# facebookresearch/lightplane

Measured on AMD Instinct MI355X. Metric: Mrays/sec fwd+bwd, 64^3x16ch triplane @128 samples; peak bwd mem (MB), higher is better.
Workload: dtype f32

## Files before the change

lightplane_amd/csrc/lp_bf3.h:

```cpp
#pragma once
#include "lp_mfma_common.h"

namespace lp {

typedef __bf16 bf16x2_t __attribute__((ext_vector_type(2)));
typedef __bf16 bf16x8_t __attribute__((ext_vector_type(8)));
typedef float f32x2_t __attribute__((ext_vector_type(2)));
typedef unsigned u32x4_t __attribute__((ext_vector_type(4)));

#define LP_MFMA_BF16(a, b, c) \
  __builtin_amdgcn_mfma_f32_32x32x16_bf16(__builtin_bit_cast(bf16x8_t, (a)), __builtin_bit_cast(bf16x8_t, (b)), (c), 0, 0, 0)

LP_DEV unsigned pk_bf16(float a, float b) {
  const f32x2_t v = {a, b};
  return __builtin_bit_cast(unsigned, __builtin_convertvector(v, bf16x2_t));
}
LP_DEV float bf16_lo(unsigned p) { return __builtin_bit_cast(float, p << 16); }
LP_DEV float bf16_hi(unsigned p) { return __builtin_bit_cast(float, p & 0xffff0000u); }

LP_DEV void split3_scalar(float x, unsigned short& l1, unsigned short& l2, unsigned short& l3) {
  const unsigned p1 = pk_bf16(x, 0.0f);
  const float r1 = x - bf16_lo(p1);
  const unsigned p2 = pk_bf16(r1, 0.0f);
  const float r2 = r1 - bf16_lo(p2);
// ... 110 lines not shown
  return acc;
}
LP_DEV void split2_chunk(const float* v, u32x4_t& l1, u32x4_t& l2) {
#pragma unroll
  for (int i = 0; i < 4; ++i) {
    const float a = v[2 * i], b = v[2 * i + 1];
    const unsigned p1 = pk_bf16(a, b);
    l1[i] = p1;
    l2[i] = pk_bf16(a - bf16_lo(p1), b - bf16_hi(p1));
  }
}
template <class A>
LP_DEV f32x16 chunk_bf2(const A& a, int c, int lane, const u32x4_t& l1, const u32x4_t& l2, f32x16 acc) {
  {
    const u32x4_t w2 = a(c, 1, lane);
    acc = LP_MFMA_BF16(w2, l1, acc);
  }
  {
    const u32x4_t w1 = a(c, 0, lane);
    acc = LP_MFMA_BF16(w1, l2, acc);
    acc = LP_MFMA_BF16(w1, l1, acc);
  }
  return acc;
}
template <int NCH, class A>
LP_DEV f32x16 layer_bf2v(const A& a, int lane, const float (&v)[8 * NCH], f32x16 acc, char* trow = nullptr) {
  u32x4_t l1, l2;
  split2_chunk(v, l1, l2);
#pragma unroll
  for (int c = 0; c < NCH; ++c) {
    u32x4_t n1 = l1, n2 = l2;
    if (trow) {
      *reinterpret_cast<u32x4_t*>(trow + 32 * c) = l1;
      *reinterpret_cast<u32x4_t*>(trow + 32 * c + rm_bytes(32)) = l2;
    }
    acc = chunk_bf2(a, c, lane, l1, l2, acc);
    if (c + 1 < NCH) split2_chunk(v + 8 * (c + 1), n1, n2);
    l1 = n1; l2 = n2;
  }
  return acc;
}
template <int NCH>
LP_DEV void limb_tile_store(char* trow, const float (&v)[8 * NCH]) {
#pragma unroll
  for (int c = 0; c < NCH; ++c) {
    u32x4_t l1, l2;
    float w[8];
#pragma unroll
    for (int i = 0; i < 8; ++i) {
      w[i] = v[8 * c + i];
      asm volatile("" : "+v"(w[i]));
    }
    split2_chunk(w, l1, l2);
    *reinterpret_cast<u32x4_t*>(trow + 32 * c) = l1;
    *reinterpret_cast<u32x4_t*>(trow + 32 * c + rm_bytes(32)) = l2;
  }
}

template <int DXL>
LP_DEV void dx_split_chunk(const float* v, u32x4_t& l1, u32x4_t& l2, u32x4_t& l3) {
  if constexpr (DXL == 2) {
    split2_chunk(v, l1, l2);
    l3 = l2;
  } else {
    split3_chunk(v, l1, l2, l3);
  }
}
template <int DXL, class A>
LP_DEV f32x16 dx_chunk(const A& a, int c, int lane, const u32x4_t& l1, const u32x4_t& l2, const u32x4_t& l3, f32x16 acc) {
  if constexpr (DXL == 2) return chunk_bf2(a, c, lane, l1, l2, acc);
  else return chunk_bf3(a, c, lane, l1, l2, l3, acc);
}
template <int NCH, int DXL = 2, class A>
LP_DEV f32x16 layer_dxv(const A& a, int lane, const float (&v)[8 * NCH], f32x16 acc, char* trow = nullptr) {
  if constexpr (DXL == 2) return layer_bf2v<NCH>(a, lane, v, acc, trow);
  else return layer_bf3v<NCH>(a, lane, v, acc);
}

template <int NCH>
LP_DEV f32x16 layer_bf3v(const char* img, int chunk0, int lane, const float (&v)[8 * NCH], f32x16 acc) {
  return layer_bf3v<NCH>(ASlots{img, chunk0}, lane, v, acc);
}

template <int NCH, class A1, class A2>
LP_DEV void layer2_bf3v(const A1& a1, const A2& a2, int lane, const float (&v)[8 * NCH], f32x16& acc_a, f32x16& acc_b) {
  u32x4_t l1, l2, l3;
  split3_chunk(v, l1, l2, l3);
#pragma unroll
  for (int c = 0; c < NCH; ++c) {
    u32x4_t n1 = l1, n2 = l2, n3 = l3;
    acc_a = chunk_bf3(a1, c, lane, l1, l2, l3, acc_a);
    acc_b = chunk_bf3(a2, c, lane, l1, l2, l3, acc_b);
    if (c + 1 < NCH) {
      split3_chunk(v + 8 * (c + 1), n1, n2, n3);
      bf3_interleave_hint();
    }
    l1 = n1; l2 = n2; l3 = n3;
  }
}
template <int NCH>
LP_DEV void layer2_bf3v(const char* img, int chunk_a, int chunk_b, int lane, const float (&v)[8 * NCH], f32x16& acc_a,
                        f32x16& acc_b) {
  layer2_bf3v<NCH>(ASlots{img, chunk_a}, ASlots{img, chunk_b}, lane, v, acc_a, acc_b);
}

template <bool FWD>
// ... 131 lines not shown
```

lightplane_amd/csrc/lp_device.h:

```cpp
#pragma once

#include <hip/hip_runtime.h>
#include <stdint.h>

#include "../../include/lightplane_hip.h"

#define LP_DEV __device__ __forceinline__

namespace lp {


struct Ray {
  float ox, oy, oz, dx, dy, dz, near_t, far_t;
  int b;
};

LP_DEV Ray load_ray(const LpRays& r, int64_t i) {
  Ray q;
  q.ox = r.origins[3 * i + 0];
  q.oy = r.origins[3 * i + 1];
  q.oz = r.origins[3 * i + 2];
  q.dx = r.directions[3 * i + 0];
  q.dy = r.directions[3 * i + 1];
  q.dz = r.directions[3 * i + 2];
// ... 308 lines not shown
    const int U = (xy || xz) ? g.W : g.H;
    const int V = xy ? g.H : g.D;
    int iu, iv;
    float wu[2], wv[2];
    bool oku[2], okv[2];
    axis_taps<SPLAT>(cu, U, iu, wu, oku);
    axis_taps<SPLAT>(cv, V, iv, wv, okv);
    t.n = 4;
    t.su = 1; t.sv = U; t.st = 0;
    t.row0 = base + iv * U + iu;
    t.iu = iu;
    t.cell = 0;
    t.ok = 0;
#pragma unroll
    for (int k = 0; k < 4; ++k) {
      const int uu = k & 1, uv = (k >> 1) & 1;
      const bool ok = oku[uu] && okv[uv];
      t.ok |= ok ? (1u << k) : 0u;
      t.w[k] = ok ? wu[uu] * wv[uv] : 0.0f;
    }
#pragma unroll
    for (int k = 4; k < 8; ++k) t.w[k] = 0.0f;
  }
}

LP_DEV float scaffold_lookup(const float* scaffold, const LpGrid& s, int b, float x, float y, float z) {
  if (!point_in_bounds(x, y, z)) return 0.0f;
  const float fx = rintf(unnormalize<false>(x, s.W));
  const float fy = rintf(unnormalize<false>(y, s.H));
  const float fz = rintf(unnormalize<false>(z, s.D));
  if (!(fx >= 0.0f && fx <= (float)(s.W - 1) && fy >= 0.0f && fy <= (float)(s.H - 1) && fz >= 0.0f &&
        fz <= (float)(s.D - 1)))
    return 0.0f;
  const int64_t row = (((int64_t)b * s.D + (int)fz) * s.H + (int)fy) * s.W + (int)fx;
  return scaffold[row];
}


LP_DEV float softplus_f(float x) {
  const float e = __expf(x);
  const float series = e * fmaf(e, fmaf(e, 0.333333343f, -0.5f), 1.0f);
  const float lg = __logf(1.0f + e);
  const float sp = (e < 0.015625f) ? series : lg;
  return (x > 20.0f) ? x : sp;
}
LP_DEV float relu_f(float x) {
  const int i = __builtin_bit_cast(int, x);
  return __builtin_bit_cast(float, i > 0 ? i : 0);
}

LP_DEV unsigned mask_bit(unsigned m, float relu_value, int q) {
  return m | ((relu_value > 0.0f) ? (1u << q) : 0u);
}
LP_DEV float mask_apply(unsigned m, int q, float v) {
  const int all = ((int)(m << (31 - q))) >> 31;
  return __builtin_bit_cast(float, __builtin_bit_cast(int, v) & all);
}

LP_DEV float sigmoid_f(float x) { return __builtin_amdgcn_rcpf(1.0f + __expf(-x)); }
LP_DEV float d_softplus_f(float x) { return (x > 20.0f) ? 1.0f : sigmoid_f(x); }


LP_DEV int32_t hash32(int32_t x) {
  x = (int32_t)((uint32_t)((x >> 16) ^ x) * 0x45D9F3Bu);
  x = (int32_t)((uint32_t)((x >> 16) ^ x) * 0x45D9F3Bu);
  return (x >> 16) ^ x;
}
LP_DEV int32_t pair_hash(int32_t x, int32_t h) {
  const uint32_t u = (uint32_t)(h ^ x);
  return (int32_t)((u << 24) + u * 0x193u);
}
LP_DEV float int32_to_u01(int32_t h) {
  return (((float)h + 2147483648.0f) + 3.0f) / 4294967296.0f;
}
LP_DEV float hash_randn(int32_t x1, int32_t x2, int32_t seed) {
  const int32_t prime = 105097564;
  const int32_t h1 = pair_hash(pair_hash(prime, seed), hash32(x1));
  const int32_t h2 = pair_hash(pair_hash(prime, seed + 1), hash32(x2));
  const float u1 = int32_to_u01(h1), u2 = int32_to_u01(h2);
  return sqrtf(-2.0f * logf(u1)) * cosf(6.28318530718f * u2);
}
LP_DEV float sample_noise(int64_t ray, int step, int64_t n_rays, int s_tot, int32_t seed) {
  const int64_t i1 = ray * s_tot + step + 1;
  const int64_t pad = n_rays > 16 ? n_rays : 16;
  const int64_t i2 = i1 + pad * s_tot;
  return hash_randn((int32_t)(uint32_t)(uint64_t)i1, (int32_t)(uint32_t)(uint64_t)i2, seed);
}

LP_DEV void write_ray_outputs(const LpRendererArgs& a, int64_t ray_id, float len, float nlt, const float* facc) {
  a.ray_length[ray_id] = len;
  a.neg_log_t[ray_id] = nlt;
  const bool epi = a.bg_color != nullptr || a.alpha != nullptr;
  const float T = epi ? expf(-nlt) : 0.0f;
  for (int c = 0; c < a.color_chn; ++c) {
    float f = facc[c];
    if (a.bg_color) f = f + T * a.bg_color[c];
    a.feature[ray_id * a.color_chn + c] = f;
  }
  if (a.alpha) a.alpha[ray_id] = (a.alpha_mode == 2) ? -nlt : 1.0f - T;
}
LP_DEV float epilogue_grad_nlt(const LpRendererArgs& a, int64_t rid, bool valid, float nlt_final, float g_nlt,
                               const float* gfeat, int n_chn) {
  if (a.bg_color == nullptr && a.grad_alpha == nullptr) return g_nlt;
  const float T = expf(-nlt_final);
  if (a.grad_alpha && valid) {
    const float ga = a.grad_alpha[rid];
// ... 20 lines not shown
```

lightplane_amd/csrc/lp_mfma_common.h:

```cpp
#pragma once
#include <stdlib.h>

#include "lp_device.h"
#include "lp_splat_walk.h"
#include "lp_host.h"
#include "lp_plane_range.h"

namespace lp {

typedef float f32x16 __attribute__((ext_vector_type(16)));

LP_DEV constexpr int featq(int q, int h) { return (q & 3) + 8 * (q >> 2) + 4 * h; }

#define LP_MFMA(a, b, c) __builtin_amdgcn_mfma_f32_32x32x2f32((a), (b), (c), 0, 0, 0)

LP_DEV int opaque_zero() {
  int z = 0;
  asm volatile("" : "+s"(z));
  return z;
}

constexpr int HID = 32;
constexpr int W_LD = 33;
constexpr int WAVES = 4;
// ... 66 lines not shown
  if (!plain || S > RANGE_MAX_S || __ballot(!valid) != 0) return w;
  const LpGrid* g = a.grid.grids;
  const int W = g[0].W, H = g[0].H, D = (GM == GM_TRIPLANE) ? g[1].D : g[0].D;
  const AxisSpans ax = ray_axis_spans(ray.ox, ray.oy, ray.oz, ray.dx, ray.dy, ray.dz, ray.near_t, ray.far_t, S, W, H, D);
#pragma unroll
  for (int p = 0; p < (GM == GM_TRIPLANE ? 3 : 1); ++p) {
    const SampleSpan sp = (GM == GM_TRIPLANE) ? plane_span(ax, p, S) : voxel_span(ax, S);
    const int lo = wave_min_i(sp.lo), hi = -wave_min_i(-sp.hi);
    if (p == 0) w.lo3 = w.hi3 = 0u;
    w.lo3 |= (unsigned)(hi < lo ? 511 : lo) << (10 * p);
    w.hi3 |= (unsigned)(hi < lo ? 0 : hi) << (10 * p);
  }
  if (GM == GM_VOXEL) {
    w.lo3 *= 0x00100401u;
    w.hi3 *= 0x00100401u;
  }
  w.lo3 = (unsigned)__builtin_amdgcn_readfirstlane((int)w.lo3);
  w.hi3 = (unsigned)__builtin_amdgcn_readfirstlane((int)w.hi3);
  return w;
}

template <int C>
LP_DEV void gather_tap(const float* data, int row, float w, int h, float (&x0)[C / 2]) {
  const float4* src = reinterpret_cast<const float4*>(data + (int64_t)(row < 0 ? 0 : row) * C + 4 * h);
#pragma unroll
  for (int j = 0; j < C / 8; ++j) {
    const float4 v = src[2 * j];
    x0[4 * j + 0] = fmaf(w, v.x, x0[4 * j + 0]);
    x0[4 * j + 1] = fmaf(w, v.y, x0[4 * j + 1]);
    x0[4 * j + 2] = fmaf(w, v.z, x0[4 * j + 2]);
    x0[4 * j + 3] = fmaf(w, v.w, x0[4 * j + 3]);
  }
}

template <int C>
LP_DEV void gather_taps4(const float* data, const int* row, const float* w, float keep, int h, float (&x0)[C / 2]) {
  float4 v[4][C / 8];
#pragma unroll
  for (int k = 0; k < 4; ++k) {
    const float4* src = reinterpret_cast<const float4*>(data + (int64_t)(row[k] < 0 ? 0 : row[k]) * C + 4 * h);
#pragma unroll
    for (int j = 0; j < C / 8; ++j) v[k][j] = src[2 * j];
  }
  __builtin_amdgcn_sched_barrier(0);
#pragma unroll
  for (int k = 0; k < 4; ++k) {
    const float wk = w[k] * keep;
#pragma unroll
    for (int j = 0; j < C / 8; ++j) {
      x0[4 * j + 0] = fmaf(wk, v[k][j].x, x0[4 * j + 0]);
      x0[4 * j + 1] = fmaf(wk, v[k][j].y, x0[4 * j + 1]);
      x0[4 * j + 2] = fmaf(wk, v[k][j].z, x0[4 * j + 2]);
      x0[4 * j + 3] = fmaf(wk, v[k][j].w, x0[4 * j + 3]);
    }
  }
}

template <int C, bool FENCED>
LP_DEV void gather_list(const LpGridList& gl, bool mask_oob, const Ray& ray, float x, float y, float z, int h,
                        float (&x0)[C / 2]) {
#pragma unroll
  for (int q = 0; q < C / 2; ++q) x0[q] = 0.0f;
  const float keep = (mask_oob && !point_in_bounds(x, y, z)) ? 0.0f : 1.0f;
  for (int g = 0; g < gl.n_grids; ++g) {
    Taps t;
    const float* data = gl.grids[g].data;
    grid_taps<false>(gl.grids[g], ray.b, x, y, z, t);
    if (FENCED) __builtin_amdgcn_sched_barrier(0);
    gather_taps4<C>(data, t.row, t.w, keep, h, x0);
    if (FENCED) __builtin_amdgcn_sched_barrier(0);
    if (t.n == 8) {
      gather_taps4<C>(data, t.row + 4, t.w + 4, keep, h, x0);
      if (FENCED) __builtin_amdgcn_sched_barrier(0);
    }
  }
}

template <int C, int GM, bool FENCED = false>
LP_DEV void gather_features(const LpRendererArgs& a, const Ray& ray, float x, float y, float z, int h,
                            float (&x0)[C / 2], unsigned pm = WaveRanges::G) {
#pragma unroll
  for (int q = 0; q < C / 2; ++q) x0[q] = 0.0f;
  const float keep = (a.march.mask_out_of_bounds && !point_in_bounds(x, y, z)) ? 0.0f : 1.0f;
  if (GM == GM_TRIPLANE) {
    if (FENCED) {
      AxisTap ax, ay, az;
      triplane_axes<false>(a.grid.grids, x, y, z, ax, ay, az);
      const int W = a.grid.grids[0].W, H = a.grid.grids[0].H, D = a.grid.grids[1].D;
#pragma unroll
      for (int g = 0; g < 3; ++g) {
        __builtin_amdgcn_sched_barrier(0);
        if (pm & WaveRanges::bit(g)) {
          Taps t;
          plane_taps_from_axes((int)a.grid.grids[g].row_offset + ray.b * ((g == 0 ? H : D) * (g == 2 ? H : W)), g == 2 ? H : W,
                               g == 2 ? ay : ax, g == 0 ? ay : az, t);
          gather_taps4<C>(a.grid.grids[g].data, t.row, t.w, keep, h, x0);
        }
      }
      __builtin_amdgcn_sched_barrier(0);
    } else {
      Taps t[3];
      triplane_taps<false>(a.grid.grids, ray.b, x, y, z, t);
#pragma unroll
      for (int g = 0; g < 3; ++g) {
        if (!(pm & WaveRanges::bit(g))) continue;
#pragma unroll
        for (int k = 0; k < 4; ++k) gather_tap<C>(a.grid.grids[g].data, t[g].row[k], t[g].w[k] * keep, h, x0);
      }
    }
  } else if (GM == GM_VOXEL) {
    if (!(pm & WaveRanges::bit(0))) return;
    Taps t;
    voxel_taps<false>(a.grid.grids[0], ray.b, x, y, z, t);
    if (FENCED) {
      __builtin_amdgcn_sched_barrier(0);
      gather_taps4<C>(a.grid.grids[0].data, t.row, t.w, keep, h, x0);
      __builtin_amdgcn_sched_barrier(0);
      gather_taps4<C>(a.grid.grids[0].data, t.row + 4, t.w + 4, keep, h, x0);
      __builtin_amdgcn_sched_barrier(0);
    } else {
#pragma unroll
      for (int k = 0; k < 8; ++k) gather_tap<C>(a.grid.grids[0].data, t.row[k], t.w[k] * keep, h, x0);
    }
  } else {
    for (int g = 0; g < a.grid.n_grids; ++g) {
      Taps t;
      const float* data = a.grid.grids[g].data;
      grid_taps<false>(a.grid.grids[g], ray.b, x, y, z, t);
      if (FENCED) {
        __builtin_amdgcn_sched_barrier(0);
        gather_taps4<C>(data, t.row, t.w, keep, h, x0);
        __builtin_amdgcn_sched_barrier(0);
        if (t.n == 8) {
          gather_taps4<C>(data, t.row + 4, t.w + 4, keep, h, x0);
          __builtin_amdgcn_sched_barrier(0);
        }
      } else {
#pragma unroll
        for (int k = 0; k < 4; ++k) gather_tap<C>(data, t.row[k], t.w[k] * keep, h, x0);
        if (t.n == 8) {
#pragma unroll
          for (int k = 4; k < 8; ++k) gather_tap<C>(data, t.row[k], t.w[k] * keep, h, x0);
        }
      }
    }
  }
}


struct Heads {
// ... 142 lines not shown
#pragma unroll
  for (int c8 = 0; c8 < 4; ++c8) {
    const float4 w0 = wsrc[2 * c8], w1 = wsrc[2 * c8 + 1];
    const float w[8] = {w0.x, w0.y, w0.z, w0.w, w1.x, w1.y, w1.z, w1.w};
    float dx[CPL][8];
#pragma unroll
    for (int j = 0; j < CPL; ++j) {
      const float4 d0 = dsrc[j][2 * c8], d1 = dsrc[j][2 * c8 + 1];
      dx[j][0] = d0.x; dx[j][1] = d0.y; dx[j][2] = d0.z; dx[j][3] = d0.w;
      dx[j][4] = d1.x; dx[j][5] = d1.y; dx[j][6] = d1.z; dx[j][7] = d1.w;
    }
#pragma unroll
    for (int i = 0; i < 8; ++i) {
      const int rr = 8 * c8 + i;
      if (rr == 0) {
#pragma unroll
        for (int j = 0; j < CPL; ++j) run[j] = 0.0f;
      } else if ((mask >> rr) & 1u) {
        flush(s_row);
#pragma unroll
        for (int j = 0; j < CPL; ++j) run[j] = 0.0f;
        s_row = __builtin_amdgcn_readlane(row0, rr);
      }
#pragma unroll
      for (int j = 0; j < CPL; ++j) run[j] = fmaf(w[i], dx[j][i], run[j]);
    }
    __builtin_amdgcn_sched_barrier(0);
  }
  flush(s_row);
}

template <int C>
LP_DEV void scatter_plane(float* gg, const LpGrid& g, int b, float x, float y, float z, bool live, int lane,
                          const float* dxT, float* wT) {
  const bool xy = g.D == 1, xz = g.H == 1;
  const float cu = (xy || xz) ? x : y;
  const float cv = xy ? y : z;
  const int U = (xy || xz) ? g.W : g.H;
  const int V = xy ? g.H : g.D;
  AxisTap u, v;
  axis_taps<false>(cu, U, u.i0, u.w, u.ok);
  axis_taps<false>(cv, V, v.i0, v.w, v.ok);
  scatter_plane_ax<C>(gg, (int)g.row_offset + b * (U * V), U, u, v, live, lane, dxT, wT);
}

struct AxisNorm {
  int i;
  float w0, w1;
  bool dead;
};
LP_DEV AxisNorm axis_norm(float c, int size) {
  AxisTap t;
  axis_taps<false>(c, size, t.i0, t.w, t.ok);
  const bool only0 = t.ok[0] & !t.ok[1], only1 = !t.ok[0] & t.ok[1];
  AxisNorm n;
  n.i = t.i0 + (only1 ? 1 : 0) - (only0 ? 1 : 0);
  n.w0 = only0 ? 0.0f : (only1 ? t.w[1] : t.w[0]);
  n.w1 = only1 ? 0.0f : (only0 ? t.w[0] : t.w[1]);
  n.dead = !(t.ok[0] | t.ok[1]);
  return n;
}
template <int C>
LP_DEV void scatter_triplane(float* const* gg_list, const LpGridList& gl, int b, float x, float y, float z, bool live, int lane,
                             const float* dxT, float* wT, unsigned pm = WaveRanges::G) {
  constexpr int CPL = C / 16;
  const int h = lane >> 5, r = lane & 31, sub = lane & 15, grp = lane >> 4;
  const int W = gl.grids[0].W, H = gl.grids[0].H, D = gl.grids[1].D;
  const AxisNorm ax = axis_norm(x, W), ay = axis_norm(y, H), az = axis_norm(z, D);
  const bool d0 = !live | ax.dead | ay.dead, d1 = !live | ax.dead | az.dead, d2 = !live | ay.dead | az.dead;
  const int row_xy = d0 ? -1 : (int)gl.grids[0].row_offset + (b * H + ay.i) * W + ax.i;
  const int row_xz = d1 ? -1 : (int)gl.grids[1].row_offset + (b * D + az.i) * W + ax.i;
  const int row_yz = d2 ? -1 : (int)gl.grids[2].row_offset + (b * D + az.i) * H + ay.i;
  const float wy = h ? ay.w1 : ay.w0, wz = h ? az.w1 : az.w0;
  float* const wl = wT + (2 * h) * 32 + r;
  wl[0] = d0 ? 0.0f : ax.w0 * wy;
  wl[32] = d0 ? 0.0f : ax.w1 * wy;
  wl[128] = d1 ? 0.0f : ax.w0 * wz;
  wl[160] = d1 ? 0.0f : ax.w1 * wz;
  wl[256] = d2 ? 0.0f : ay.w0 * wz;
  wl[288] = d2 ? 0.0f : ay.w1 * wz;
  const bool first = r == 0;
  const unsigned m_xy = (unsigned)__builtin_amdgcn_readfirstlane((int)(unsigned)__ballot(first | (row_xy != lane_prev(row_xy))));
  const unsigned m_xz = (unsigned)__builtin_amdgcn_readfirstlane((int)(unsigned)__ballot(first | (row_xz != lane_prev(row_xz))));
  const unsigned m_yz = (unsigned)__builtin_amdgcn_readfirstlane((int)(unsigned)__ballot(first | (row_yz != lane_prev(row_yz))));
  const float4* dsrc[CPL];
#pragma unroll
  for (int j = 0; j < CPL; ++j) dsrc[j] = reinterpret_cast<const float4*>(dxT + (sub + 16 * j) * DX_LD);
#pragma unroll 1
  for (int g = 0; g < 3; ++g) {
    if (!(pm & WaveRanges::bit(g))) continue;
    const int row0 = g == 0 ? row_xy : (g == 1 ? row_xz : row_yz);
    const unsigned mask = g == 0 ? m_xy : (g == 1 ? m_xz : m_yz);
    const int U = g == 2 ? H : W;
    const float4* wsrc = reinterpret_cast<const float4*>(wT + g * 128 + grp * 32);
    const int koff = (grp & 1) + (grp >> 1) * U;
    const unsigned lane_off = (unsigned)koff * (unsigned)(C * 4) + (unsigned)(sub * 4);
    float* const gg = gg_list[g];
    float run[CPL];
    int s_row = __builtin_amdgcn_readlane(row0, 0);
    auto flush = [&](int row) {
      if (row >= 0) {
        char* rb = reinterpret_cast<char*>(gg) + (int64_t)row * (C * 4);
#pragma unroll
        for (int j = 0; j < CPL; ++j) atomic_add_f32(reinterpret_cast<float*>(rb + lane_off + 64 * j), run[j]);
      }
    };
    if (mask == 1u) {
#pragma unroll
      for (int j = 0; j < CPL; ++j) run[j] = 0.0f;
#pragma unroll
      for (int c4 = 0; c4 < 8; ++c4) {
        const float4 w = wsrc[c4];
#pragma unroll
        for (int j = 0; j < CPL; ++j) {
          const float4 d = dsrc[j][c4];
          run[j] = fmaf(w.x, d.x, run[j]);
          run[j] = fmaf(w.y, d.y, run[j]);
          run[j] = fmaf(w.z, d.z, run[j]);
          run[j] = fmaf(w.w, d.w, run[j]);
        }
      }
      flush(s_row);
      continue;
    }
#pragma unroll
    for (int c8 = 0; c8 < 4; ++c8) {
      const float4 w0 = wsrc[2 * c8], w1 = wsrc[2 * c8 + 1];
      const float w[8] = {w0.x, w0.y, w0.z, w0.w, w1.x, w1.y, w1.z, w1.w};
      float dx[CPL][8];
#pragma unroll
      for (int j = 0; j < CPL; ++j) {
        const float4 d0v = dsrc[j][2 * c8], d1v = dsrc[j][2 * c8 + 1];
        dx[j][0] = d0v.x; dx[j][1] = d0v.y; dx[j][2] = d0v.z; dx[j][3] = d0v.w;
// ... 125 lines not shown
```

lightplane_amd/csrc/lp_renderer_mfma_bwd.h:

```cpp
#pragma once
#include "lp_mfma_common.h"
#include <type_traits>

#include "lp_bf3.h"

namespace lp {

#ifdef LP_ASM_MARKS
#define LP_MARK(n) asm volatile("; LPMARK " n)
#else
#define LP_MARK(n)
#endif
typedef float f32x4 __attribute__((ext_vector_type(4)));
#define LP_MFMA16(a, b, c) __builtin_amdgcn_mfma_f32_16x16x4f32((a), (b), (c), 0, 0, 0)

constexpr int T_LD = 36;

LP_DEV constexpr int pi16(int m) { return m < 4 ? 2 * m : (m < 12 ? 2 * (m - 4) + 1 : 2 * (m - 8)); }

LP_DEV void lds_barrier() { asm volatile("s_waitcnt lgkmcnt(0)\n\ts_barrier" ::: "memory"); }

LP_DEV void tile_store_fm(float* tile, int r, int h, const float (&v)[16]) {
#pragma unroll
  for (int q = 0; q < 16; ++q) tile[featq(q, h) * T_LD + r] = v[q];
// ... 144 lines not shown
    }
  }
  float dsum[16];
#pragma unroll
  for (int q = 0; q < 16; ++q) dsum[q] = 0.0f;
  float gfeat[4];
#pragma unroll
  for (int c = 0; c < 4; ++c)
    gfeat[c] = (valid && a.grad_feature && c < a.color_chn) ? a.grad_feature[rid * a.color_chn + c] : 0.0f;
  const float g_len = (valid && a.grad_ray_length) ? a.grad_ray_length[rid] : 0.0f;
  const float g_nlt = epilogue_grad_nlt(a, rid, valid, a.neg_log_t[rid],
                                        (valid && a.grad_neg_log_t) ? a.grad_neg_log_t[rid] : 0.0f, gfeat, 4);
  const bool want_params = a.grad_mlp_params != nullptr;
  const float delta0 = (a.march.num_samples > 1) ? (ray.far_t - ray.near_t) / (float)(a.march.num_samples - 1) : 1.0f;

  const int mi = (wave & 3) >> 1, ni = wave & 1;
  const int v0 = 4 * (wave >> 2);
  const int m16 = lane & 15, ka = lane >> 4;
  const int a_off = B::XT + (16 * mi + pi16(m16)) * T_LD + 8 * ka;
  const int b_off = B::YT + (16 * ni + pi16(m16)) * T_LD + 8 * ka;
  auto rho = [](int k) { return (k & 0x15) | ((k & 2) << 2) | ((k & 8) >> 2); };
  char* const xrow = reinterpret_cast<char*>(wv) + B::XT * 4 + rm_off(rho(r), 4 * h);
  char* const yrow = xrow + (B::YT - B::XT) * 4;
  const int xq_off = B::XT * 4 + rm_off(rho(8 * ka + (m16 >> 2)), 4 * (m16 & 3)) + 32 * mi;
  const int yq_off = B::YT * 4 + rm_off(rho(8 * ka + (m16 >> 2)), 4 * (m16 & 3)) + 32 * ni;
  f32x4 dq_b = {0, 0, 0, 0};
  auto onehot = [&](int li) -> unsigned { return (lane & 15) == li ? 0x3F803F80u : 0u; };
  const int a_off_t1 = (C == 16) ? B::XT + pi16(m16) * T_LD + 8 * ka : a_off;
  const int t1_v0 = (C == 16) ? 2 * (wave >> 1) : v0, t1_v1 = (C == 16) ? 2 * (wave >> 1) + 2 : v0 + 4;
  f32x4 dq_t1 = {0, 0, 0, 0}, dq_t2 = {0, 0, 0, 0}, dq_o1 = {0, 0, 0, 0}, dq_c1 = {0, 0, 0, 0};
  float db_t1 = 0.0f, db_t2 = 0.0f, db_o1 = 0.0f, db_c1 = 0.0f;
  float dwo2 = 0.0f, dwc2[4] = {0.0f, 0.0f, 0.0f, 0.0f};
  float dbo2 = 0.0f, dbc2[4] = {0.0f, 0.0f, 0.0f, 0.0f};
  const bool gg = a.grad_grid_list[0] != nullptr;

  float nlt = a.neg_log_t[rid];
  float suffix = 0.0f, p_next = 0.0f;
  if (seg_on) {
    const float4* pj = reinterpret_cast<const float4*>(a.seg_prefix + (rid * n_rec + s_begin / LP_SEG_LEN) * 8);
    const float4* pt = reinterpret_cast<const float4*>(a.seg_prefix + (rid * n_rec + n_rec - 1) * 8);
    const float4 j0 = pj[0], j1 = pj[1], t0 = pt[0];
    nlt = j1.y;
    nlt_lo = j1.z;
    if (seg < n_seg - 1) {
      float rest = g_len * (t0.x - j0.x);
      rest = fmaf(gfeat[0], t0.y - j0.y, rest);
      rest = fmaf(gfeat[1], t0.z - j0.z, rest);
      rest = fmaf(gfeat[2], t0.w - j0.w, rest);
      if (NC == 4) rest = fmaf(gfeat[3], pt[1].x - j1.x, rest);
      suffix = -rest;
    }
  }
  const WaveRanges rg = wave_plane_ranges<GM>(a, ray, valid, PLAIN && !SEG);
  Sample<C> nx;
  fetch_sample<C, GM, false, PLAIN>(a, sm, ray, s_begin, h, nx);
  for (int s = s_begin; s >= s_lo; --s) {
    const bool on = PLAIN || s <= s_last_w;
    const unsigned pm = rg.mask(s);
    const bool ggs = gg && pm != 0u;
    const float depth = nx.depth, occ = nx.occ, x = nx.x, y = nx.y, z = nx.z;
    float x0[C / 2];
#pragma unroll
    for (int q = 0; q < C / 2; ++q) x0[q] = nx.x0[q];
    const int zo = opaque_zero();
    const float* ldz = sm + zo;
    auto Af = [&](auto layer) {
      constexpr int l = decltype(layer)::value;
      if constexpr (NW == 8) return ASlots{fimg + zo, l == 0 ? L::CH_T1 : l == 1 ? L::CH_T2 : l == 2 ? L::CH_O1 : L::CH_C1};
      else return AColsFwd{rimg + zo + (l == 0 ? R::L_T1 : l == 1 ? R::L_T2 : l == 2 ? R::L_O1 : R::L_C1), l == 0 ? R::ST_T1 : R::ST_32};
    };
    auto Ab = [&](auto layer) {
      constexpr int l = decltype(layer)::value;
      if constexpr (NW == 8) return ASlots{bimg + zo, l == 0 ? L::CB_T1 : l == 1 ? L::CB_T2 : l == 2 ? L::CB_O1 : L::CB_C1};
      else return ARowsBwd{rimg + zo + (l == 0 ? R::L_T1 : l == 1 ? R::L_T2 : l == 2 ? R::L_O1 : R::L_C1), l == 0 ? R::ST_T1 : R::ST_32,
                           l == 0 ? C - 1 : 31};
    };
    using I0 = std::integral_constant<int, 0>; using I1 = std::integral_constant<int, 1>;
    using I2 = std::integral_constant<int, 2>; using I3 = std::integral_constant<int, 3>;

    LP_MARK("fwd");
    float h1[16];
    float e[16];
    unsigned ho_mask = 0, hc_mask = 0;
    Heads hd;
    {
      f32x16 acc;
      {
        acc = layer_bf3v<C / 16>(Af(I0{}), lane, x0, load_bias(sm, 0, h, zo));
#pragma unroll
        for (int q = 0; q < 16; ++q) h1[q] = relu_f(acc[q]);
      }
      acc = layer_bf3v<2>(Af(I1{}), lane, h1, load_bias(sm, 1, h, zo));
#pragma unroll
      for (int q = 0; q < 16; ++q) {
        e[q] = relu_f(acc[q]);
      }
      float ho[16], hc[16];
      {
        f32x16 acc_o = load_bias(sm, 2, h, zo), acc_c;
        if (CBL) {
#pragma unroll
          for (int i = 0; i < 4; ++i) {
            const float4 v = *reinterpret_cast<const float4*>(cbt + zo + ((i + cb_rot) & 3) * 4);
            acc_c[4 * i] = v.x; acc_c[4 * i + 1] = v.y; acc_c[4 * i + 2] = v.z; acc_c[4 * i + 3] = v.w;
          }
        } else {
#pragma unroll
          for (int q = 0; q < 16; ++q) acc_c[q] = cb[q];
        }
        layer2_bf3v<2>(Af(I2{}), Af(I3{}), lane, e, acc_o, acc_c);
#pragma unroll
        for (int q = 0; q < 16; ++q) {
          ho[q] = relu_f(acc_o[q]);
          hc[q] = relu_f(acc_c[q]);
        }
      }
      hd = heads_forward<NC>(sm, h, ho, hc, zo);
#pragma unroll
      for (int q = 0; q < 16; ++q) {
        ho_mask = mask_bit(ho_mask, ho[q], q);
        hc_mask = mask_bit(hc_mask, hc[q], q);
      }
      if constexpr (DUMP) {
        unsigned m1 = 0, m2 = 0, mo = 0, mc = 0;
#pragma unroll
        for (int q = 0; q < 16; ++q) {
          const unsigned bit = 1u << featq(q, h);
          m1 |= (h1[q] > 0.0f) ? bit : 0u;
          m2 |= (e[q] > 0.0f) ? bit : 0u;
          mo |= ((ho_mask >> q) & 1u) ? bit : 0u;
          mc |= ((hc_mask >> q) & 1u) ? bit : 0u;
        }
        m1 |= __shfl_xor(m1, 32); m2 |= __shfl_xor(m2, 32); mo |= __shfl_xor(mo, 32); mc |= __shfl_xor(mc, 32);
        if (valid && h == 0) {
          uint32_t* d = mp.relu_dump + (rid * s_tot + s) * 5;
          d[0] = m1; d[1] = m2; d[2] = mo; d[3] = mc; d[4] = on ? 1u : 2u;
        }
      }
      LP_SCHED_FENCE();
      if (want_params) {
        tile_store_fm(xt, r, h, ho);
        tile_store_fm(yt, r, h, hc);
      }
      LP_SCHED_FENCE();
    }

    LP_MARK("compositing");
    const float depth_prev =
        PLAIN ? ray.near_t + lin01((s > 0) ? s - 1 : 0, a.march.num_samples) * (ray.far_t - ray.near_t)
              : sample_depth_tab((s > 0) ? s - 1 : 0, a.march, ray.near_t, ray.far_t, sm + M::INF);
    const float delta = (s == 0) ? delta0 : depth - depth_prev;
    float raw = hd.raw_o;
    if (!PLAIN && a.noise_sigma > 0.0f)
      raw = raw + sample_noise(rid, s, a.rays.n_rays, s_tot, a.noise_seed) * a.noise_sigma;
    const float opacity = a.gain * softplus_f(raw) * occ;
    if (on && a.neg_log_t_ckpt) {
      const int ck = PLAIN ? ((((s + 1) % LP_NLT_CKPT) == 0 || s == s_tot - 1) ? s / LP_NLT_CKPT : -1)
                           : ckpt_index(s, a.march);
      if (ck >= 0) {
        const float2 c2 = *reinterpret_cast<const float2*>(a.neg_log_t_ckpt + (rid * n_ckpt + ck) * 2);
        nlt = c2.x;
        nlt_lo = c2.y;
      }
    }
    const float t_i = __expf(-nlt);
    nlt_add(nlt, nlt_lo, on ? -(opacity * delta) : 0.0f);
    if (!(nlt > 0.0f)) { nlt = 0.0f; nlt_lo = 0.0f; }
    const float t_im1 = __expf(-nlt);
    const float w = t_im1 - t_i;
    float sg[4];
    float p_i = g_len * depth;
#pragma unroll
    for (int c = 0; c < 4; ++c) {
      sg[c] = (c < NC) ? sigmoid_f(hd.raw_c[c]) : 0.0f;
      if (c < NC) p_i = fmaf(gfeat[c], sg[c] * occ, p_i);
    }
    suffix = on ? fmaf(t_i, p_i - p_next, suffix) : suffix;
    p_next = on ? p_i : p_next;
    const float d_a = suffix + g_nlt;
    const bool contrib = valid && on;
    const float dro = contrib ? d_a * delta * a.gain * occ * d_softplus_f(raw) : 0.0f;
    float drc[4];
#pragma unroll
    for (int c = 0; c < 4; ++c) drc[c] = (c < NC && contrib) ? w * gfeat[c] * occ * sg[c] * (1.0f - sg[c]) : 0.0f;

    LP_MARK("heads_bwd");
    float dhc[16];
    {
      const float* wc2 = sm + M::WC2 + 16 * h + opaque_zero();
#pragma unroll
      for (int j = 0; j < 4; ++j) {
#pragma unroll
        for (int i = 0; i < 4; ++i) {
          const int q = 4 * j + i;
          const float4 wc = *reinterpret_cast<const float4*>(wc2 + (8 * j + i) * 4);
          float v = drc[0] * wc.x;
          v = fmaf(drc[1], wc.y, v);
          v = fmaf(drc[2], wc.z, v);
          if (NC > 3) v = fmaf(drc[3], wc.w, v);
          dhc[q] = mask_apply(hc_mask, q, v);
        }
        LP_SCHED_FENCE();
      }
    }
    if (h == 0) {
      dbo2 += dro;
#pragma unroll
      for (int c = 0; c < NC; ++c) dbc2[c] += drc[c];
    }
    if (want_params) {
      if (h == 0) {
        ts[r] = dro;
#pragma unroll
        for (int c = 0; c < NC; ++c) ts[(1 + c) * 32 + r] = drc[c];
      }
      const float* xf = xt + r * T_LD + 16 * h;
      const float* yf = yt + r * T_LD + 16 * h;
      const float* tf = ts + 16 * h;
#pragma unroll
      for (int i = 0; i < 4; ++i) {
        const float4 hov = *reinterpret_cast<const float4*>(xf + 4 * i);
        const float4 hcv = *reinterpret_cast<const float4*>(yf + 4 * i);
        const float4 d0 = *reinterpret_cast<const float4*>(tf + 4 * i);
        dwo2 = fmaf(hov.x, d0.x, dwo2); dwo2 = fmaf(hov.y, d0.y, dwo2);
        dwo2 = fmaf(hov.z, d0.z, dwo2); dwo2 = fmaf(hov.w, d0.w, dwo2);
#pragma unroll
        for (int c = 0; c < NC; ++c) {
          const float4 dc = *reinterpret_cast<const float4*>(tf + (1 + c) * 32 + 4 * i);
          dwc2[c] = fmaf(hcv.x, dc.x, dwc2[c]); dwc2[c] = fmaf(hcv.y, dc.y, dwc2[c]);
          dwc2[c] = fmaf(hcv.z, dc.z, dwc2[c]); dwc2[c] = fmaf(hcv.w, dc.w, dwc2[c]);
        }
        LP_SCHED_FENCE();
      }
    }
    LP_SCHED_FENCE();

    LP_MARK("c1");
#ifndef LP_NO_PRIO
    __builtin_amdgcn_s_setprio(1);
#endif
    f32x16 acc = (f32x16){0};
    {
      if constexpr (DWB) {
        if (want_params) limb_tile_store<2>(xrow, e);
        acc = layer_dxv<2, DXL>(Ab(I3{}), lane, dhc, acc, want_params ? yrow : nullptr);
      } else {
        if (want_params) {
          tile_store_fm(xt, r, h, e);
          tile_store_fm(yt, r, h, dhc);
        }
        acc = layer_dxv<2, DXL>(Ab(I3{}), lane, dhc, acc);
      }
#pragma unroll
      for (int q = 0; q < 16; ++q) dsum[q] += dhc[q];
      if (want_params) {
        lds_barrier();
        if constexpr (DWB) dq_c1 = dw_quadrant_bf<B::PER_WAVE * 4>(reinterpret_cast<const char*>(wave0), xq_off, yq_off, v0, v0 + 4, dq_c1, dq_b, onehot(0));
        else dq_c1 = dw_quadrant<B::PER_WAVE>(wave0, a_off, b_off, v0, v0 + 4, dq_c1, db_c1);
        lds_barrier();
      }
    }
    LP_SCHED_FENCE();
    LP_MARK("o1");
    {
      float dho[16];
#pragma unroll
      for (int j = 0; j < 4; ++j) {
        const float4 wo = *reinterpret_cast<const float4*>(ldz + M::WO2 + 8 * j + 4 * h);
        dho[4 * j + 0] = mask_apply(ho_mask, 4 * j + 0, dro * wo.x);
        dho[4 * j + 1] = mask_apply(ho_mask, 4 * j + 1, dro * wo.y);
        dho[4 * j + 2] = mask_apply(ho_mask, 4 * j + 2, dro * wo.z);
        dho[4 * j + 3] = mask_apply(ho_mask, 4 * j + 3, dro * wo.w);
      }
      if constexpr (DWB) {
        acc = layer_dxv<2, DXL>(Ab(I2{}), lane, dho, acc, want_params ? yrow : nullptr);
      } else {
        if (want_params) tile_store_fm(yt, r, h, dho);
        acc = layer_dxv<2, DXL>(Ab(I2{}), lane, dho, acc);
      }
      if (want_params) {
        lds_barrier();
        if constexpr (DWB) dq_o1 = dw_quadrant_bf<B::PER_WAVE * 4>(reinterpret_cast<const char*>(wave0), xq_off, yq_off, v0, v0 + 4, dq_o1, dq_b, onehot(1));
        else dq_o1 = dw_quadrant<B::PER_WAVE>(wave0, a_off, b_off, v0, v0 + 4, dq_o1, db_o1);
        lds_barrier();
      }
    }
    float de[16];
#pragma unroll
    for (int q = 0; q < 16; ++q) de[q] = (e[q] > 0.0f) ? acc[q] : 0.0f;
    LP_SCHED_FENCE();
    LP_MARK("t2");
    float dh1[16];
    {
      if constexpr (DWB) {
        if (want_params) limb_tile_store<2>(xrow, h1);
        acc = layer_dxv<2, DXL>(Ab(I1{}), lane, de, (f32x16){0}, want_params ? yrow : nullptr);
      } else {
        if (want_params) {
          tile_store_fm(xt, r, h, h1);
          tile_store_fm(yt, r, h, de);
        }
        acc = layer_dxv<2, DXL>(Ab(I1{}), lane, de, (f32x16){0});
      }
      if (want_params) {
        lds_barrier();
        if constexpr (DWB) dq_t2 = dw_quadrant_bf<B::PER_WAVE * 4>(reinterpret_cast<const char*>(wave0), xq_off, yq_off, v0, v0 + 4, dq_t2, dq_b, onehot(2));
        else dq_t2 = dw_quadrant<B::PER_WAVE>(wave0, a_off, b_off, v0, v0 + 4, dq_t2, db_t2);
      }
#pragma unroll
      for (int q = 0; q < 16; ++q) dh1[q] = (h1[q] > 0.0f) ? acc[q] : 0.0f;
      if (want_params) lds_barrier();
    }
    LP_SCHED_FENCE();
    LP_MARK("t1");
    {
      if constexpr (DWB) {
        if (want_params) limb_tile_store<C / 16>(xrow, x0);
        if (ggs) {
          acc = layer_dxv<2, DXL>(Ab(I0{}), lane, dh1, (f32x16){0}, want_params ? yrow : nullptr);
        } else if (want_params) {
          limb_tile_store<2>(yrow, dh1);
        }
      } else {
        if (want_params) {
#pragma unroll
          for (int q = 0; q < C / 2; ++q) xt[featq(q, h) * T_LD + r] = x0[q];
          tile_store_fm(yt, r, h, dh1);
        }
        if (ggs) {
          acc = layer_dxv<2, DXL>(Ab(I0{}), lane, dh1, (f32x16){0});
        }
      }
      if (want_params) {
        lds_barrier();
        if constexpr (DWB) dq_t1 = dw_quadrant_bf<B::PER_WAVE * 4>(reinterpret_cast<const char*>(wave0), (C == 16) ? xq_off - 32 * mi : xq_off, yq_off, t1_v0, t1_v1, dq_t1, dq_b, onehot(3));
        else dq_t1 = dw_quadrant<B::PER_WAVE>(wave0, a_off_t1, b_off, t1_v0, t1_v1, dq_t1, db_t1);
        lds_barrier();
      }
    }
    if (ggs) {
#pragma unroll
      for (int q = 0; q < C / 2; ++q) xt[featq(q, h) * DX_LD + r] = acc[q];
    }
    LP_SCHED_FENCE();
    LP_MARK("fetch");
    __builtin_amdgcn_s_setprio(0);
    const bool live = valid && on && !(a.march.mask_out_of_bounds && !point_in_bounds(x, y, z));
    if (s > s_lo) fetch_sample<C, GM, true, PLAIN>(a, sm, ray, s - 1, h, nx, rg.mask(s - 1));
    LP_SCHED_FENCE();
    LP_MARK("scatter");
    if (ggs) {
      if constexpr (GM == GM_TRIPLANE) {
        scatter_triplane<C>(a.grad_grid_list, a.grid, ray.b, x, y, z, live, lane, xt, yt, pm);
      } else {
        const int ng = (GM == GM_VOXEL) ? 1 : a.grid.n_grids;
#pragma unroll 1
        for (int g = 0; g < ng; ++g)
          scatter_grid<C, GM>(a.grad_grid_list[g], a.grid.grids[g], ray.b, x, y, z, live, lane, xt, yt);
      }
    }
  }

  LP_MARK("epilogue");
  {
    f32x16 acc;
    if constexpr (NW == 8) acc = layer_bf3v<2>(ASlots{bimg, L::CB_C1}, lane, dsum, (f32x16){0});
    else acc = layer_bf3v<2>(ARowsBwd{rimg + R::L_C1, R::ST_32, 31}, lane, dsum, (f32x16){0});
    if (valid && a.grad_encoding && !seg_on) {
      float4* dst = reinterpret_cast<float4*>(a.grad_encoding + ray_id * HID + 4 * h);
#pragma unroll
      for (int j = 0; j < 4; ++j) dst[2 * j] = make_float4(acc[4 * j], acc[4 * j + 1], acc[4 * j + 2], acc[4 * j + 3]);
    } else if (valid && a.grad_encoding) {
      float* dst = a.grad_encoding + ray_id * HID + 4 * h;
#pragma unroll
// ... 141 lines not shown
```

Before: 30.69.

## Micro-optimize backward: packed bf16 cvt, bitfield mask gating, clamped plane taps, carried transmittance

Several unrelated instruction-level tweaks land in the backward renderer and gather paths. Limb tile stores now split with a direct v_cvt_pk_bf16_f32 and a single residual conversion. The ReLU output mask is built by shifting and tested with v_bfe_i32. The fenced triplane gather clamps indices and zeroes weights instead of building per-tap rows with -1 sentinels, and axis normalisation is made branch-free. The transmittance exp from the previous step is also carried over to drop one __expf per sample. Each change trims ALU work, at the cost of inline asm that limits the compiler and a changed mask bit order that the dump path has to mirror.

```diff
diff --git a/lightplane_amd/csrc/lp_bf3.h b/lightplane_amd/csrc/lp_bf3.h
--- a/lightplane_amd/csrc/lp_bf3.h
+++ b/lightplane_amd/csrc/lp_bf3.h
@@ -186,6 +186,27 @@
       asm volatile("" : "+v"(w[i]));
     }
     split2_chunk(w, l1, l2);
+    *reinterpret_cast<u32x4_t*>(trow + 32 * c) = l1;
+    *reinterpret_cast<u32x4_t*>(trow + 32 * c + rm_bytes(32)) = l2;
+  }
+}
+LP_DEV unsigned pk_bf16_opaque(float a, float b) {
+  unsigned p;
+  asm volatile("v_cvt_pk_bf16_f32 %0, %1, %2" : "=v"(p) : "v"(a), "v"(b));
+  return p;
+}
+template <int NCH>
+LP_DEV void limb_tile_store_cvt(char* trow, const float (&v)[8 * NCH]) {
+#pragma unroll
+  for (int c = 0; c < NCH; ++c) {
+    u32x4_t l1, l2;
+#pragma unroll
+    for (int i = 0; i < 4; ++i) {
+      const float a = v[8 * c + 2 * i], b = v[8 * c + 2 * i + 1];
+      const unsigned p1 = pk_bf16_opaque(a, b);
+      l1[i] = p1;
+      l2[i] = pk_bf16(a - bf16_lo(p1), b - bf16_hi(p1));
+    }
     *reinterpret_cast<u32x4_t*>(trow + 32 * c) = l1;
     *reinterpret_cast<u32x4_t*>(trow + 32 * c + rm_bytes(32)) = l2;
   }
diff --git a/lightplane_amd/csrc/lp_device.h b/lightplane_amd/csrc/lp_device.h
--- a/lightplane_amd/csrc/lp_device.h
+++ b/lightplane_amd/csrc/lp_device.h
@@ -384,6 +384,13 @@
 LP_DEV unsigned mask_bit(unsigned m, float relu_value, int q) {
   return m | ((relu_value > 0.0f) ? (1u << q) : 0u);
 }
+LP_DEV unsigned mask_push(unsigned m, float relu_value) { return m + m + ((relu_value > 0.0f) ? 1u : 0u); }
+template <int Q>
+LP_DEV float mask_gate(unsigned m, float v) {
+  int all;
+  asm("v_bfe_i32 %0, %1, %2, 1" : "=v"(all) : "v"(m), "n"(Q));
+  return __builtin_bit_cast(float, __builtin_bit_cast(int, v) & all);
+}
 LP_DEV float mask_apply(unsigned m, int q, float v) {
   const int all = ((int)(m << (31 - q))) >> 31;
   return __builtin_bit_cast(float, __builtin_bit_cast(int, v) & all);
diff --git a/lightplane_amd/csrc/lp_mfma_common.h b/lightplane_amd/csrc/lp_mfma_common.h
--- a/lightplane_amd/csrc/lp_mfma_common.h
+++ b/lightplane_amd/csrc/lp_mfma_common.h
@@ -142,6 +142,43 @@
       x0[4 * j + 1] = fmaf(wk, v[k][j].y, x0[4 * j + 1]);
       x0[4 * j + 2] = fmaf(wk, v[k][j].z, x0[4 * j + 2]);
       x0[4 * j + 3] = fmaf(wk, v[k][j].w, x0[4 * j + 3]);
+    }
+  }
+}
+
+struct AxisClamp {
+  int i[2];
+  float w[2];
+};
+LP_DEV AxisClamp axis_clamp(const AxisTap& t, int size) {
+  AxisClamp c;
+  c.i[0] = min(max(t.i0, 0), size - 1);
+  c.i[1] = min(max(t.i0 + 1, 0), size - 1);
+  c.w[0] = t.ok[0] ? t.w[0] : 0.0f;
+  c.w[1] = t.ok[1] ? t.w[1] : 0.0f;
+  return c;
+}
+template <int C>
+LP_DEV void gather_plane_clamped(const float* data, int base, int U, const AxisClamp& u, const AxisClamp& v, float keep, int h,
+                                 float (&x0)[C / 2]) {
+  float4 val[4][C / 8];
+#pragma unroll
+  for (int k = 0; k < 4; ++k) {
+    const unsigned row = (unsigned)(base + v.i[k >> 1] * U + u.i[k & 1]);
+    const float4* src = reinterpret_cast<const float4*>(data + (uint64_t)row * C + 4 * h);
+#pragma unroll
+    for (int j = 0; j < C / 8; ++j) val[k][j] = src[2 * j];
+  }
+  __builtin_amdgcn_sched_barrier(0);
+#pragma unroll
+  for (int k = 0; k < 4; ++k) {
+    const float wk = (u.w[k & 1] * v.w[k >> 1]) * keep;
+#pragma unroll
+    for (int j = 0; j < C / 8; ++j) {
+      x0[4 * j + 0] = fmaf(wk, val[k][j].x, x0[4 * j + 0]);
+      x0[4 * j + 1] = fmaf(wk, val[k][j].y, x0[4 * j + 1]);
+      x0[4 * j + 2] = fmaf(wk, val[k][j].z, x0[4 * j + 2]);
+      x0[4 * j + 3] = fmaf(wk, val[k][j].w, x0[4 * j + 3]);
     }
   }
 }
@@ -177,15 +214,13 @@
       AxisTap ax, ay, az;
       triplane_axes<false>(a.grid.grids, x, y, z, ax, ay, az);
       const int W = a.grid.grids[0].W, H = a.grid.grids[0].H, D = a.grid.grids[1].D;
+      const AxisClamp cx = axis_clamp(ax, W), cy = axis_clamp(ay, H), cz = axis_clamp(az, D);
 #pragma unroll
       for (int g = 0; g < 3; ++g) {
         __builtin_amdgcn_sched_barrier(0);
-        if (pm & WaveRanges::bit(g)) {
-          Taps t;
-          plane_taps_from_axes((int)a.grid.grids[g].row_offset + ray.b * ((g == 0 ? H : D) * (g == 2 ? H : W)), g == 2 ? H : W,
-                               g == 2 ? ay : ax, g == 0 ? ay : az, t);
-          gather_taps4<C>(a.grid.grids[g].data, t.row, t.w, keep, h, x0);
-        }
+        if (pm & WaveRanges::bit(g))
+          gather_plane_clamped<C>(a.grid.grids[g].data, (int)a.grid.grids[g].row_offset + ray.b * ((g == 0 ? H : D) * (g == 2 ? H : W)),
+                                  g == 2 ? H : W, g == 2 ? cy : cx, g == 0 ? cy : cz, keep, h, x0);
       }
       __builtin_amdgcn_sched_barrier(0);
     } else {
@@ -434,11 +469,12 @@
 LP_DEV AxisNorm axis_norm(float c, int size) {
   AxisTap t;
   axis_taps<false>(c, size, t.i0, t.w, t.ok);
-  const bool only0 = t.ok[0] & !t.ok[1], only1 = !t.ok[0] & t.ok[1];
+  const bool swap = t.ok[0] != t.ok[1];
+  const float g0 = t.ok[0] ? t.w[0] : 0.0f, g1 = t.ok[1] ? t.w[1] : 0.0f;
   AxisNorm n;
-  n.i = t.i0 + (only1 ? 1 : 0) - (only0 ? 1 : 0);
-  n.w0 = only0 ? 0.0f : (only1 ? t.w[1] : t.w[0]);
-  n.w1 = only1 ? 0.0f : (only0 ? t.w[0] : t.w[1]);
+  n.i = min(max(t.i0, 0), size - 2);
+  n.w0 = swap ? g1 : g0;
+  n.w1 = swap ? g0 : g1;
   n.dead = !(t.ok[0] | t.ok[1]);
   return n;
 }
@@ -453,14 +489,14 @@
   const int row_xy = d0 ? -1 : (int)gl.grids[0].row_offset + (b * H + ay.i) * W + ax.i;
   const int row_xz = d1 ? -1 : (int)gl.grids[1].row_offset + (b * D + az.i) * W + ax.i;
   const int row_yz = d2 ? -1 : (int)gl.grids[2].row_offset + (b * D + az.i) * H + ay.i;
-  const float wy = h ? ay.w1 : ay.w0, wz = h ? az.w1 : az.w0;
+  const float wy = live ? (h ? ay.w1 : ay.w0) : 0.0f, wz = live ? (h ? az.w1 : az.w0) : 0.0f;
   float* const wl = wT + (2 * h) * 32 + r;
-  wl[0] = d0 ? 0.0f : ax.w0 * wy;
-  wl[32] = d0 ? 0.0f : ax.w1 * wy;
-  wl[128] = d1 ? 0.0f : ax.w0 * wz;
-  wl[160] = d1 ? 0.0f : ax.w1 * wz;
-  wl[256] = d2 ? 0.0f : ay.w0 * wz;
-  wl[288] = d2 ? 0.0f : ay.w1 * wz;
+  wl[0] = ax.w0 * wy;
+  wl[32] = ax.w1 * wy;
+  wl[128] = ax.w0 * wz;
+  wl[160] = ax.w1 * wz;
+  wl[256] = ay.w0 * wz;
+  wl[288] = ay.w1 * wz;
   const bool first = r == 0;
   const unsigned m_xy = (unsigned)__builtin_amdgcn_readfirstlane((int)(unsigned)__ballot(first | (row_xy != lane_prev(row_xy))));
   const unsigned m_xz = (unsigned)__builtin_amdgcn_readfirstlane((int)(unsigned)__ballot(first | (row_xz != lane_prev(row_xz))));
diff --git a/lightplane_amd/csrc/lp_renderer_mfma_bwd.h b/lightplane_amd/csrc/lp_renderer_mfma_bwd.h
--- a/lightplane_amd/csrc/lp_renderer_mfma_bwd.h
+++ b/lightplane_amd/csrc/lp_renderer_mfma_bwd.h
@@ -220,6 +220,7 @@
     }
   }
   const WaveRanges rg = wave_plane_ranges<GM>(a, ray, valid, PLAIN && !SEG);
+  float t_carry = __expf(-nlt);
   Sample<C> nx;
   fetch_sample<C, GM, false, PLAIN>(a, sm, ray, s_begin, h, nx);
   for (int s = s_begin; s >= s_lo; --s) {
@@ -286,9 +287,10 @@
       hd = heads_forward<NC>(sm, h, ho, hc, zo);
 #pragma unroll
       for (int q = 0; q < 16; ++q) {
-        ho_mask = mask_bit(ho_mask, ho[q], q);
+        ho_mask = mask_push(ho_mask, ho[q]);
         hc_mask = mask_bit(hc_mask, hc[q], q);
       }
+      asm volatile("" : "+v"(ho_mask));
       if constexpr (DUMP) {
         unsigned m1 = 0, m2 = 0, mo = 0, mc = 0;
 #pragma unroll
@@ -296,7 +298,7 @@
           const unsigned bit = 1u << featq(q, h);
           m1 |= (h1[q] > 0.0f) ? bit : 0u;
           m2 |= (e[q] > 0.0f) ? bit : 0u;
-          mo |= ((ho_mask >> q) & 1u) ? bit : 0u;
+          mo |= ((ho_mask >> (15 - q)) & 1u) ? bit : 0u;
           mc |= ((hc_mask >> q) & 1u) ? bit : 0u;
         }
         m1 |= __shfl_xor(m1, 32); m2 |= __shfl_xor(m2, 32); mo |= __shfl_xor(mo, 32); mc |= __shfl_xor(mc, 32);
@@ -329,12 +331,14 @@
         const float2 c2 = *reinterpret_cast<const float2*>(a.neg_log_t_ckpt + (rid * n_ckpt + ck) * 2);
         nlt = c2.x;
         nlt_lo = c2.y;
-      }
-    }
-    const float t_i = __expf(-nlt);
+        t_carry = __expf(-nlt);
+      }
+    }
+    const float t_i = t_carry;
     nlt_add(nlt, nlt_lo, on ? -(opacity * delta) : 0.0f);
     if (!(nlt > 0.0f)) { nlt = 0.0f; nlt_lo = 0.0f; }
     const float t_im1 = __expf(-nlt);
+    t_carry = t_im1;
     const float w = t_im1 - t_i;
     float sg[4];
     float p_i = g_len * depth;
@@ -410,7 +414,7 @@
     f32x16 acc = (f32x16){0};
     {
       if constexpr (DWB) {
-        if (want_params) limb_tile_store<2>(xrow, e);
+        if (want_params) limb_tile_store_cvt<2>(xrow, e);
         acc = layer_dxv<2, DXL>(Ab(I3{}), lane, dhc, acc, want_params ? yrow : nullptr);
       } else {
         if (want_params) {
@@ -432,14 +436,15 @@
     LP_MARK("o1");
     {
       float dho[16];
-#pragma unroll
-      for (int j = 0; j < 4; ++j) {
+      auto gate4 = [&](auto jc) {
+        constexpr int j = decltype(jc)::value;
         const float4 wo = *reinterpret_cast<const float4*>(ldz + M::WO2 + 8 * j + 4 * h);
-        dho[4 * j + 0] = mask_apply(ho_mask, 4 * j + 0, dro * wo.x);
-        dho[4 * j + 1] = mask_apply(ho_mask, 4 * j + 1, dro * wo.y);
-        dho[4 * j + 2] = mask_apply(ho_mask, 4 * j + 2, dro * wo.z);
-        dho[4 * j + 3] = mask_apply(ho_mask, 4 * j + 3, dro * wo.w);
-      }
+        dho[4 * j + 0] = mask_gate<15 - (4 * j + 0)>(ho_mask, dro * wo.x);
+        dho[4 * j + 1] = mask_gate<15 - (4 * j + 1)>(ho_mask, dro * wo.y);
+        dho[4 * j + 2] = mask_gate<15 - (4 * j + 2)>(ho_mask, dro * wo.z);
+        dho[4 * j + 3] = mask_gate<15 - (4 * j + 3)>(ho_mask, dro * wo.w);
+      };
+      gate4(I0{}); gate4(I1{}); gate4(I2{}); gate4(I3{});
       if constexpr (DWB) {
         acc = layer_dxv<2, DXL>(Ab(I2{}), lane, dho, acc, want_params ? yrow : nullptr);
       } else {
@@ -461,7 +466,7 @@
     float dh1[16];
     {
       if constexpr (DWB) {
-        if (want_params) limb_tile_store<2>(xrow, h1);
+        if (want_params) limb_tile_store_cvt<2>(xrow, h1);
         acc = layer_dxv<2, DXL>(Ab(I1{}), lane, de, (f32x16){0}, want_params ? yrow : nullptr);
       } else {
         if (want_params) {
@@ -483,11 +488,11 @@
     LP_MARK("t1");
     {
       if constexpr (DWB) {
-        if (want_params) limb_tile_store<C / 16>(xrow, x0);
+        if (want_params) limb_tile_store_cvt<C / 16>(xrow, x0);
         if (ggs) {
           acc = layer_dxv<2, DXL>(Ab(I0{}), lane, dh1, (f32x16){0}, want_params ? yrow : nullptr);
         } else if (want_params) {
-          limb_tile_store<2>(yrow, dh1);
+          limb_tile_store_cvt<2>(yrow, dh1);
         }
       } else {
         if (want_params) {
```

Result: faster. 31.25, median of 6 (+1.8%).
